# scheckmedia/centernet-uda

Hardware: AMD Instinct MI355X
Metric: images/sec CenterNet DLA-34 512x512 UDA step (entropy minimisation) (higher is better)
Workload: dtype f32; 1 GPU; configs[2]: DLA-34 + DCNv2, 512x512, per-GPU batch 16 source + 16 target, uda=entropy_minimization, Adam(lr 5e-5), random-init weights; global_batch=16, parallelism=dp1

## Files before the change

### centernet-uda_amd/csrc/dcn.hip

```cpp
#include <algorithm>
#include "igemm.cuh"
#include "igemm_host.h"

namespace cnuda {
namespace {

struct DcnGeom {
    int B, C, H, W, Co, kh, kw, sh, sw, ph, pw, dh, dw, dg, Ho, Wo;
    int off_bs, mask_bs, goff_bs, gmask_bs, gmask_logit;
};

struct Tap {
    int o00, o01, o10, o11;
    int h0, w0;
    float lh, lw, hh, hw;
    float mask;
    bool inside, c00, c01, c10, c11;
};

struct TapRaw { float dy, dx, mask; };
__device__ __forceinline__ TapRaw load_tap_raw(const DcnGeom& g, const float* __restrict__ off_b,
                                               const float* __restrict__ mask_b, int grp, int tap, int p) {
    const int T = g.kh * g.kw, HoWo = g.Ho * g.Wo;
    TapRaw r;
// ... 167 lines not shown
            if (k < K) {
                const int tap = k / g.C, c = k - tap * g.C;
                if (tap != cur) set_tap(tap);
                v = sample(in_b + (size_t)c * HW);
            }
            r.t[j].l = v;
        }
    }
    __device__ __forceinline__ void finish(const Raw& r, float (&v)[8]) {
        if (!r.eager) {
            if (!r.live) {
#pragma unroll
                for (int j = 0; j < 8; ++j) v[j] = 0.0f;
                return;
            }
#pragma unroll
            for (int j = 0; j < 8; ++j) v[j] = m00 * r.t[j].l + m01 * r.t[j].r + m10 * r.b[j].l + m11 * r.b[j].r;
            if constexpr (BUF) {
                if (col_on && col_voff != IG_BUF_OOB) {
                    const int k0s = __builtin_amdgcn_readfirstlane(r.k0);
                    const char* cbase = reinterpret_cast<const char*>(col_base);
                    unsigned voff = col_voff;
                    asm volatile("" : "+v"(voff));
#pragma unroll
                    for (int j = 0; j < 8; ++j) {
                        const size_t row = (size_t)(unsigned)((k0s + 2 * j) * col_stride) * 4u;
                        unsigned long long rbase = reinterpret_cast<unsigned long long>(cbase) + row;
                        asm volatile("" : "+s"(rbase));
                        *reinterpret_cast<__attribute__((address_space(1))) float*>(rbase + (unsigned long long)voff) = v[j];
                    }
                }
                return;
            }
            if (col_n) {
                float* cp = col_n + (size_t)r.k0 * col_stride;
                const size_t step = (size_t)2 * col_stride;
#pragma unroll
                for (int j = 0; j < 8; ++j) cp[j * step] = v[j];
            }
            return;
        }
#pragma unroll
        for (int j = 0; j < 8; ++j) {
            const int k = r.k0 + 2 * j;
            v[j] = r.t[j].l;
            if (col_n && k < K) col_n[(size_t)k * col_stride] = v[j];
        }
    }
    struct Out {
        float* base;
        int HoWo;
        __device__ Out(const Params& p, long long n) {
            HoWo = p.g.Ho * p.g.Wo;
            const int ni = (int)n, b = ni / HoWo, pp = ni - b * HoWo;
            base = p.out + (size_t)b * p.g.Co * HoWo + pp;
        }
        __device__ __forceinline__ void store(const Params& p, int m, float v) {
            v += p.bias[m];
            if (p.act_slope >= 0.0f && v < 0.0f) v *= p.act_slope;
            base[(size_t)m * HoWo] = v;
        }
        static constexpr bool kVec4 = true;
        __device__ static bool vec4_ok(const Params& p) { return ((p.g.Ho * p.g.Wo) & 3) == 0; }
        __device__ __forceinline__ void store4(const Params& p, int m, f32x4 v) {
            v += p.bias[m];
            if (p.act_slope >= 0.0f) {
#pragma unroll
                for (int e = 0; e < 4; ++e) if (v[e] < 0.0f) v[e] *= p.act_slope;
            }
            *reinterpret_cast<f32x4*>(base + (size_t)m * HoWo) = v;
        }
    };
};

using DcnFwdLoader = DcnFwdLoaderT<false>;
using DcnFwdBufLoader = DcnFwdLoaderT<true>;

constexpr int DW_MARGIN = 3;
typedef __attribute__((address_space(3))) volatile unsigned char lds_vu8;
template <int TC> struct DwTile {
    static constexpr int TR = IG_BN / TC, NR = TR + 2 + 2 * DW_MARGIN, RS = TC + 8, PL = NR * RS;
    static constexpr int CPR = TC / 4 + 2, CPP = NR * CPR, CELLS = 16 * CPP;
    static constexpr int NCELL = (CELLS + IG_THREADS - 1) / IG_THREADS;
    static constexpr int SHIFT = TC == 32 ? 5 : 4;
};
template <int TC> constexpr size_t dcnw_lds_floats(int bm) { return (size_t)16 * DwTile<TC>::PL + 2 * IG_KC * bm; }

template <int BM, int TC>
__global__ __launch_bounds__(IG_THREADS, 3) void dcnw_fwd_kernel(DcnFwdParams p, const float* __restrict__ A, int Mp, int Kp,
                                                                 int n_tiles, int tiles_x) {
    using Q = DwTile<TC>;
    constexpr int TM = BM / 32, PL = Q::PL, RS = Q::RS;
    extern __shared__ __attribute__((aligned(16))) float smem[];
    const DcnGeom& g = p.g;
    const int W = g.W, H = g.H, HW = g.H * g.W;
    float* const Hs = smem;
    float* const Asb = smem + 16 * PL;
    const int tid = threadIdx.x, lane = tid & 63, wid = tid >> 6;
    int tile = xcd_remap(blockIdx.x, n_tiles);
    const int tile_id = tile;
    const int tx = tile % tiles_x; tile /= tiles_x;
    const int tiles_y = H / Q::TR;
    const int ty = tile % tiles_y, b = tile / tiles_y;
    const int y0 = ty * Q::TR, x0 = tx * TC;
    const int yw0 = y0 - 1 - DW_MARGIN;
    const int pxl = wid * 32 + (lane & 31), kl = lane >> 5;
    const int py = y0 + (pxl >> Q::SHIFT), px = x0 + (pxl & (TC - 1)), pp = py * W + px;

    const buf_rsrc rs = ig_make_rsrc(p.in, (unsigned)((size_t)g.B * g.C * HW * sizeof(float)));
    auto cell = [&](int i, unsigned& voff, int& loff) {
        int salt = 0;
        asm volatile("" : "+v"(salt));
        const int e = tid + i * IG_THREADS + salt;
        const int c = e / Q::CPP, rem = e - c * Q::CPP;
        const int row = rem / Q::CPR, q4 = rem - row * Q::CPR;
        const int iy = yw0 + row, ix = x0 - 4 + 4 * q4;
        loff = e < Q::CELLS ? c * PL + row * RS + 4 * q4 : -1;
        voff = (e < Q::CELLS && iy >= 0 && iy < H && ix >= 0 && ix < W)
                   ? (unsigned)(((b * g.C + c) * HW + iy * W + ix) * (int)sizeof(float)) : IG_BUF_OOB;
    };

    int addr[9];
    float flh[9], flw[9], fmk[9];
    unsigned stray = 0;
    {
        const float* off_b = p.off + (size_t)b * g.off_bs + pp;
        const float* mask_b = p.mask + (size_t)b * g.mask_bs + pp;
        float dy[9], dx[9], mk[9];
#pragma unroll
        for (int t = 0; t < 9; ++t) {
            dy[t] = off_b[(size_t)(2 * t) * HW];
            dx[t] = off_b[(size_t)(2 * t + 1) * HW];
            mk[t] = mask_b[(size_t)t * HW];
        }
#pragma unroll
        for (int t = 0; t < 9; ++t) {
            const float h = (float)(py - 1 + t / 3) + dy[t], w = (float)(px - 1 + t % 3) + dx[t];
            const float hf = floorf(h), wf = floorf(w);
            const bool valid = h > -1.0f && w > -1.0f && h < (float)H && w < (float)W;
            const int h0 = valid ? (int)hf : 0, w0i = valid ? (int)wf : 0;
            const int wr = h0 - yw0, wc = w0i - x0 + 4;
            const bool inwin = valid && wr >= 0 && wr + 1 <= Q::NR - 1 && wc >= 0 && wc + 1 <= RS - 1;
            addr[t] = inwin ? wr * RS + wc : 0;
            flh[t] = h - hf;
            flw[t] = w - wf;
            fmk[t] = inwin ? mk[t] : 0.0f;
            if (valid && !inwin) stray |= 1u << t;
        }
    }
    const bool any_stray = __any(stray != 0);

    f32x16 acc[TM];
#pragma unroll
    for (int i = 0; i < TM; ++i)
#pragma unroll
        for (int r = 0; r < 16; ++r) acc[i][r] = 0.0f;

    f32x4 hreg[Q::NCELL];
    auto win_load = [&](int grp) {
        const unsigned soff = (unsigned)(grp * 16 * HW) * (unsigned)sizeof(float);
#pragma unroll
        for (int i = 0; i < Q::NCELL; ++i) {
            unsigned voff; int loff;
            cell(i, voff, loff);
            hreg[i] = ig_buf_load4(rs, voff, soff);
        }
    };
    auto win_store = [&]() {
#pragma unroll
        for (int i = 0; i < Q::NCELL; ++i) {
            unsigned voff; int loff;
            cell(i, voff, loff);
            if (loff >= 0) *reinterpret_cast<f32x4*>(Hs + loff) = hreg[i];
        }
    };
    f32x4 ra[ig_a_per<BM>()];
    const IgABuf<BM> abuf(A, Mp, Kp, 0, tid);
    const int nchunk = Kp / IG_KC, G = g.C >> 4;
    const bool col_on = p.col != nullptr;
    float* const col_l = col_on ? p.col + (size_t)b * 9 * g.C * HW + (size_t)kl * HW + pp : nullptr;

    win_load(0);
    abuf.load(0, ra);
    win_store();
    ig_store_a<BM>(Asb, tid, ra);
    if (1 < nchunk) abuf.load(IG_KC, ra);
    __syncthreads();
    int grp = 0;
    for (int c0 = 0; c0 < nchunk; c0 += 9, ++grp) {
        const bool more = grp + 1 < G;
        if (more) win_load(grp + 1);
#pragma unroll
        for (int t = 0; t < 9; ++t) {
            const int c = c0 + t;
            f32x4 ra2[ig_a_per<BM>()];
            if (c + 2 < nchunk) abuf.load((c + 2) * IG_KC, ra2);
            const float* As = Asb + (c & 1) * IG_KC * BM;
            const float* ap = As + kl * BM + (lane & 31);
            int a_t = addr[t];
            asm volatile("" : "+v"(a_t));
            const float* hb = Hs + kl * PL + a_t;
            const float lh = flh[t], lw = flw[t], hh = 1.0f - lh, hw = 1.0f - lw, mk = fmk[t];
            const float w00 = hh * hw * mk, w01 = hh * lw * mk, w10 = lh * hw * mk, w11 = lh * lw * mk;
            float v[IG_KC / 2], cr[IG_KC / 4][4];
            float* cp = nullptr;
            if (col_on) {
                unsigned long long rowoff = (unsigned long long)(unsigned)((t * g.C + grp * 16) * HW) * sizeof(float);
                asm volatile("" : "+s"(rowoff));
                cp = reinterpret_cast<float*>(reinterpret_cast<char*>(col_l) + rowoff);
            }
            auto read_half = [&](int h) {
#pragma unroll
                for (int s = 0; s < IG_KC / 4; ++s) {
                    const float* q = hb + 2 * (h * (IG_KC / 4) + s) * PL;
                    cr[s][0] = q[0]; cr[s][1] = q[1]; cr[s][2] = q[RS]; cr[s][3] = q[RS + 1];
                }
            };
            auto blend_half = [&](int h) {
#pragma unroll
                for (int s = 0; s < IG_KC / 4; ++s) {
                    float x = w00 * cr[s][0];
                    x = fmaf(w01, cr[s][1], x);
                    x = fmaf(w10, cr[s][2], x);
                    v[h * (IG_KC / 4) + s] = fmaf(w11, cr[s][3], x);
                }
                if (col_on) {
#pragma unroll
                    for (int s = 0; s < IG_KC / 4; ++s) cp[(size_t)(2 * (h * (IG_KC / 4) + s)) * HW] = v[h * (IG_KC / 4) + s];
                }
            };
            auto mma_half = [&](int h) {
#pragma unroll
                for (int s = h * (IG_KC / 4); s < (h + 1) * (IG_KC / 4); ++s) {
#pragma unroll
                    for (int i = 0; i < TM; ++i)
                        acc[i] = __builtin_amdgcn_mfma_f32_32x32x2f32(ap[2 * s * BM + i * 32], v[s], acc[i], 0, 0, 0);
                }
            };
            read_half(0);
            blend_half(0);
            read_half(1);
            __builtin_amdgcn_sched_barrier(0);
            mma_half(0);
            __builtin_amdgcn_sched_barrier(0);
            blend_half(1);
            mma_half(1);
            if (c + 1 < nchunk) ig_store_a<BM>(Asb + ((c + 1) & 1) * IG_KC * BM, tid, ra);
#pragma unroll
            for (int i = 0; i < ig_a_per<BM>(); ++i) ra[i] = ra2[i];
            __syncthreads();
            __builtin_amdgcn_sched_barrier(0);
        }
        if (any_stray) {
#pragma unroll 1
            for (int t0 = 0; t0 < 9; ++t0) {
                int t = t0;
                asm volatile("" : "+s"(t));
                if (!__any((stray >> t) & 1u)) continue;
                float sv[IG_KC / 2];
#pragma unroll
                for (int s = 0; s < IG_KC / 2; ++s) sv[s] = 0.0f;
                if ((stray >> t) & 1u) {
                    const float* off_b = p.off + (size_t)b * g.off_bs + pp;
                    const int tr = t / 3;
                    const float sh_ = (float)(py - 1 + tr) + off_b[(size_t)(2 * t) * HW];
                    const float sw_ = (float)(px - 1 + t - 3 * tr) + off_b[(size_t)(2 * t + 1) * HW];
                    const float smk = p.mask[(size_t)b * g.mask_bs + (size_t)t * HW + pp];
                    const float shf = floorf(sh_), swf = floorf(sw_);
                    const int sh0 = (int)shf, sw0 = (int)swf;
                    const float slh = sh_ - shf, slw = sw_ - swf, shh = 1.0f - slh, shw = 1.0f - slw;
                    const bool top = sh0 >= 0, bot = sh0 + 1 <= H - 1, lef = sw0 >= 0, rig = sw0 + 1 <= W - 1;
                    const float g00 = (top && lef) ? shh * shw * smk : 0.0f, g01 = (top && rig) ? shh * slw * smk : 0.0f;
                    const float g10 = (bot && lef) ? slh * shw * smk : 0.0f, g11 = (bot && rig) ? slh * slw * smk : 0.0f;
                    const int cy0 = top ? sh0 : 0, cy1 = bot ? sh0 + 1 : H - 1, cx0 = lef ? sw0 : 0, cx1 = rig ? sw0 + 1 : W - 1;
                    const float* in_c = p.in + ((size_t)b * g.C + grp * 16 + kl) * HW;
                    const int o00 = cy0 * W + cx0, o01 = cy0 * W + cx1, o10 = cy1 * W + cx0, o11 = cy1 * W + cx1;
#pragma unroll
                    for (int s = 0; s < IG_KC / 2; ++s) {
                        const float* pl = in_c + (size_t)(2 * s) * HW;
                        float x = g00 * pl[o00];
                        x = fmaf(g01, pl[o01], x);
                        x = fmaf(g10, pl[o10], x);
                        sv[s] = fmaf(g11, pl[o11], x);
                    }
                    if (col_on) {
                        float* cp = col_l + (size_t)(t * g.C + grp * 16) * HW;
#pragma unroll
                        for (int s = 0; s < IG_KC / 2; ++s) cp[(size_t)(2 * s) * HW] = sv[s];
                    }
                }
                const float* ag = A + (size_t)((c0 + t) * IG_KC + kl) * Mp + (lane & 31);
#pragma unroll
                for (int s = 0; s < IG_KC / 2; ++s) {
#pragma unroll
                    for (int i = 0; i < TM; ++i)
                        acc[i] = __builtin_amdgcn_mfma_f32_32x32x2f32(ag[(size_t)(2 * s) * Mp + i * 32], sv[s], acc[i], 0, 0, 0);
                }
            }
        }
        if (more) {
            win_store();
            __syncthreads();
        }
    }
    float* stage = smem + wid * IG_EPI_WAVE;
    const int col = lane & 31, cg = lane & 7, rsub = lane >> 3;
    const int epl = wid * 32 + 4 * cg;
    float* const obase = p.out + (size_t)b * g.Co * HW + (size_t)(y0 + (epl >> Q::SHIFT)) * W + x0 + (epl & (TC - 1));
#pragma unroll
    for (int i = 0; i < TM; ++i) {
#pragma unroll
        for (int r = 0; r < 16; ++r) stage[mfma_row(r, lane) * IG_EPI_LD + col] = acc[i][r];
        asm volatile("s_waitcnt lgkmcnt(0)" ::: "memory");
#pragma unroll
        for (int it = 0; it < 4; ++it) {
            const int row = it * 8 + rsub;
            f32x4 v4 = *reinterpret_cast<const f32x4*>(stage + row * IG_EPI_LD + 4 * cg);
            const int m = i * 32 + row;
            if (m < g.Co) {
                v4 += p.bias[m];
                if (p.act_slope >= 0.0f) {
#pragma unroll
                    for (int e = 0; e < 4; ++e) if (v4[e] < 0.0f) v4[e] *= p.act_slope;
                }
                *reinterpret_cast<f32x4*>(obase + (size_t)m * HW) = v4;
            }
            if (p.stats) {
                float s1 = (v4[0] + v4[1]) + (v4[2] + v4[3]);
                float s2 = (v4[0] * v4[0] + v4[1] * v4[1]) + (v4[2] * v4[2] + v4[3] * v4[3]);
                auto row8 = [](float v) {
                    v += __builtin_bit_cast(float, __builtin_amdgcn_update_dpp(0, __builtin_bit_cast(int, v), 0xB1, 0xf, 0xf, false));
                    v += __builtin_bit_cast(float, __builtin_amdgcn_update_dpp(0, __builtin_bit_cast(int, v), 0x4E, 0xf, 0xf, false));
                    v += __builtin_bit_cast(float, __builtin_amdgcn_update_dpp(0, __builtin_bit_cast(int, v), 0x141, 0xf, 0xf, false));
                    return v;
                };
                s1 = row8(s1);
                s2 = row8(s2);
                if (cg == 0)
                    reinterpret_cast<float2*>(p.stats)[((size_t)tile_id * 4 + wid) * p.stats_mp + m] = make_float2(s1, s2);
            }
        }
        asm volatile("s_waitcnt lgkmcnt(0)" ::: "memory");
    }
}

struct DcnSampleParams {
    DcnGeom g;
    const float *in, *off, *mask;
    float* col;
};
__global__ __launch_bounds__(1024) void dcn_sample_kernel(DcnSampleParams p, int tiles_per_image) {
    const DcnGeom& g = p.g;
    const int T = g.kh * g.kw, HoWo = g.Ho * g.Wo, HW = g.H * g.W;
    const int b = blockIdx.x / tiles_per_image, tile = blockIdx.x - b * tiles_per_image;
    const int px = tile * 64 + threadIdx.x;
    if (px >= HoWo) return;
    const int oy = px / g.Wo, ox = px - oy * g.Wo;
    const float* in_b = p.in + (size_t)b * g.C * HW;
    for (int tap = threadIdx.y; tap < T; tap += blockDim.y) {
        const Tap t = make_tap(g, p.off + (size_t)b * g.off_bs, p.mask + (size_t)b * g.mask_bs, 0, tap, oy, ox);
        const float mk = t.inside ? t.mask : 0.0f;
        const float w00 = t.c00 ? t.hh * t.hw * mk : 0.0f, w01 = t.c01 ? t.hh * t.lw * mk : 0.0f;
        const float w10 = t.c10 ? t.lh * t.hw * mk : 0.0f, w11 = t.c11 ? t.lh * t.lw * mk : 0.0f;
        float* dst = p.col + ((size_t)b * T + tap) * g.C * HoWo + px;
        const bool paired = g.W >= 2;
        const bool ledge = t.w0 < 0, redge = t.w0 > g.W - 2;
        const int wa = ledge ? 0 : (redge ? g.W - 2 : t.w0);
        const int ht = t.h0 < 0 ? 0 : t.h0, hb = t.h0 + 1 > g.H - 1 ? g.H - 1 : t.h0 + 1;
        const int qT = t.inside ? ht * g.W + wa : 0, qB = t.inside ? hb * g.W + wa : 0;
        for (int c0 = 0; c0 < g.C; c0 += 8) {
            float e00[8], e01[8], e10[8], e11[8];
            if (paired) {
                Pair pt[8], pb[8];
#pragma unroll
                for (int u = 0; u < 8; ++u) {
                    const float* plane = in_b + (size_t)(c0 + u < g.C ? c0 + u : g.C - 1) * HW;
                    pt[u] = *reinterpret_cast<const Pair*>(plane + qT);
                    pb[u] = *reinterpret_cast<const Pair*>(plane + qB);
                }
#pragma unroll
                for (int u = 0; u < 8; ++u) {
                    e00[u] = redge ? pt[u].r : pt[u].l; e01[u] = ledge ? pt[u].l : pt[u].r;
                    e10[u] = redge ? pb[u].r : pb[u].l; e11[u] = ledge ? pb[u].l : pb[u].r;
                }
            } else {
#pragma unroll
                for (int u = 0; u < 8; ++u) {
                    const float* plane = in_b + (size_t)(c0 + u < g.C ? c0 + u : g.C - 1) * HW;
                    e00[u] = plane[t.o00]; e01[u] = plane[t.o01]; e10[u] = plane[t.o10]; e11[u] = plane[t.o11];
                }
// ... 924 lines not shown
}

extern "C" int cnuda_dcn_v2_forward(const float* input, const float* weight, const float* bias, const float* offset,
                                    const float* mask, float* output, int B, int C, int H, int W, int Cout, int kh,
                                    int kw, int sh, int sw, int ph, int pw, int dh, int dw, int dg, void* workspace,
                                    size_t workspace_bytes, cnuda_stream_t stream) {
    return cnuda_dcn_v2_forward_cols(input, weight, bias, offset, mask, output, nullptr, B, C, H, W, Cout, kh, kw, sh,
                                     sw, ph, pw, dh, dw, dg, workspace, workspace_bytes, stream);
}

extern "C" int cnuda_dcn_v2_forward_cols(const float* input, const float* weight, const float* bias,
                                         const float* offset, const float* mask, float* output, float* columns, int B,
                                         int C, int H, int W, int Cout, int kh, int kw, int sh, int sw, int ph, int pw,
                                         int dh, int dw, int dg, void* workspace, size_t workspace_bytes,
                                         cnuda_stream_t stream) {
    return cnuda_dcn_v2_forward_act(input, weight, bias, offset, mask, output, columns, -1.0f, B, C, H, W, Cout, kh, kw,
                                    sh, sw, ph, pw, dh, dw, dg, workspace, workspace_bytes, stream);
}

extern "C" int cnuda_dcn_v2_stats_block(int B, int C, int H, int W, int Cout, int kh, int kw, int sh, int sw, int ph, int pw,
                                        int dh, int dw, int dg, int* rows) {
    DcnGeom g;
    if (fill_geom(g, B, C, H, W, Cout, kh, kw, sh, sw, ph, pw, dh, dw, dg, "cnuda_dcn_v2_stats_block")) return 0;
    return plan_stats_block(g, make_plan(g), rows);
}

static int dcn_forward_impl(const DcnFwdCall& c, const DcnPlan& q) {
    const DcnGeom& g = c.g;
    CNUDA_REQUIRE(c.input && c.weight && c.bias && c.offset && c.mask && c.output, "cnuda_dcn_v2_forward: null pointer");
    CNUDA_REQUIRE(!c.columns || g.W >= 2, "cnuda_dcn_v2_forward_cols: columns output needs width >= 2");
    hipStream_t st = (hipStream_t)c.stream;
    CNUDA_REQUIRE(c.act_slope < 0.0f || (g.dg == 1 && g.W >= 2), "cnuda_dcn_v2_forward_act: fused activation needs deformable_group == 1 and width >= 2");
    if (q.fwd == DcnFwdPath::Composed) {
        const int Cg = g.C / g.dg, T = q.T, HoWo = g.Ho * g.Wo;
        const long long HW = (long long)g.H * g.W;
        const size_t inner = cnuda_dcn_v2_workspace_bytes(g.B, Cg, g.H, g.W, g.Co, g.kh, g.kw, g.sh, g.sw, g.ph, g.pw, g.dh, g.dw, 1);
        Carver cv(c.workspace, c.workspace_bytes);
        float* xg = cv.take<float>((size_t)g.B * Cg * HW);
        float* wg = cv.take<float>((size_t)g.Co * Cg * T);
        float* tmp = cv.take<float>((size_t)g.B * g.Co * HoWo);
        float* zero = cv.take<float>((size_t)g.Co);
        void* iws = cv.take<char>(inner);
        CNUDA_REQUIRE(c.workspace && cv.cur <= cv.end, "cnuda_dcn_v2_forward: workspace too small");
        if (hipMemsetAsync(zero, 0, (size_t)g.Co * sizeof(float), st) != hipSuccess) return check_launch("cnuda_dcn_v2_forward(dg>1)");
        DcnFwdCall gc = c;
        gc.g.C = Cg; gc.g.dg = 1;
        gc.input = xg; gc.weight = wg;
        gc.workspace = iws; gc.workspace_bytes = inner;
        const DcnPlan gq = make_plan(gc.g);
        const PackStampSuspend uncached;
        for (int grp = 0; grp < g.dg; ++grp) {
            if (int rc = cnuda_copy_channels(c.input, xg, g.B, Cg, HW, g.C, grp * Cg, Cg, 0, c.stream)) return rc;
            if (int rc = cnuda_copy_channels(c.weight, wg, g.Co, Cg, T, g.C, grp * Cg, Cg, 0, c.stream)) return rc;
            gc.bias = grp == 0 ? c.bias : zero;
            gc.offset = c.offset + (size_t)grp * 2 * T * HoWo;
            gc.mask = c.mask + (size_t)grp * T * HoWo;
            gc.output = grp == 0 ? c.output : tmp;
            gc.columns = c.columns ? c.columns + (size_t)grp * g.B * T * Cg * HoWo : nullptr;
            if (int rc = dcn_forward_impl(gc, gq)) return rc;
            if (grp > 0)
                if (int rc = cnuda_add(c.output, tmp, c.output, (long long)g.B * g.Co * HoWo, c.stream)) return rc;
        }
        return check_launch("cnuda_dcn_v2_forward(dg>1)");
    }
    if (q.fwd == DcnFwdPath::Naive) {
        DcnNaiveParams p{g, c.input, c.weight, c.bias, c.offset, c.mask, nullptr, c.output, nullptr, nullptr, nullptr, nullptr};
        CNUDA_LAUNCH(dcn_naive_fwd_kernel, dim3(stream_grid((long long)g.B * g.Co * g.Ho * g.Wo, 256)), dim3(256),
                           0, st, p);
        return check_launch("cnuda_dcn_v2_forward(dg>1)");
    }
    CNUDA_REQUIRE(q.N < (1ll << 31) - IG_BN, "cnuda_dcn_v2_forward: more than 2^31 pixels per call");
    CNUDA_REQUIRE(c.workspace && c.workspace_bytes >= q.fwd_bytes, "cnuda_dcn_v2_forward: workspace too small");
    Carver cv(c.workspace, c.workspace_bytes);
    if (q.fwd == DcnFwdPath::Window) {
        const int bm = 64;
        const float* Aw = launch_pack(c.weight, cv.take<float>((size_t)q.Kp * bm), (size_t)q.Kp * bm * sizeof(float), g.Co, g.C,
                                      q.T, PACK_HALO_FWD, q.Kp, bm, 0, st);
        DcnFwdParams p{g, c.input, c.offset, c.mask, c.bias, c.act_slope, c.output, c.columns, c.stats, 64};
        ProfScope prof(st);
        prof.name("dcnw_fwd_kernel<%d>%s", bm, c.columns ? " (+ column side output)" : "");
        const int tiles_x = g.W / dcnw_tile_cols(g.W), n_tiles = (int)(q.N / IG_BN);
        bool lds_ok = true;
        const bool found = with_tiles<Tile<64, 32>, Tile<64, 16>>(bm, dcnw_tile_cols(g.W), [&](auto BM, auto TC) {
            const size_t fl = dcnw_lds_floats<TC()>(BM());
            const size_t lds = (fl < (size_t)4 * IG_EPI_WAVE ? (size_t)4 * IG_EPI_WAVE : fl) * sizeof(float);
            lds_ok = raise_dynamic_lds(reinterpret_cast<const void*>(&dcnw_fwd_kernel<BM(), TC()>), lds);
            if (lds_ok) CNUDA_LAUNCH((dcnw_fwd_kernel<BM(), TC()>), dim3(n_tiles), dim3(IG_THREADS), lds, st, p, Aw, bm, q.Kp, n_tiles, tiles_x);
        });
        CNUDA_REQUIRE(lds_ok, "cnuda_dcn_v2_forward: dynamic LDS");
        CNUDA_REQUIRE(found, "cnuda_dcn_v2_forward: no dcnw_fwd_kernel instance for %d-column tiles", dcnw_tile_cols(g.W));
        return check_launch("cnuda_dcn_v2_forward(window)");
    }
    const float* A = launch_pack(c.weight, cv.take<float>((size_t)q.Kp * q.Mp), (size_t)q.Kp * q.Mp * sizeof(float), g.Co,
                                 g.C, q.T, PACK_FWD, q.Kp, q.Mp, 0, st);
    if (q.fwd == DcnFwdPath::SampleThenGemm) {
        float* cols = c.columns ? c.columns : cv.take<float>((size_t)g.B * q.K * g.Ho * g.Wo);
        ProfScope prof(st);
        prof.name("dcn_sample_kernel + igemm_fwd_kernel<%d, DcnColsLoader>", q.bm);
        {
            DcnSampleParams sp{g, c.input, c.offset, c.mask, cols};
            const int tiles = ceil_div(g.Ho * g.Wo, 64), tw = q.T < 16 ? q.T : 16;
            CNUDA_LAUNCH(dcn_sample_kernel, dim3(g.B * tiles), dim3(64, tw), 0, st, sp, tiles);
        }
        DcnColsParams p{g, cols, c.bias, c.act_slope, c.output, c.stats, q.Mp};
        const bool found = q.fwd_ws    ? launch_dcn_fwd<DcnColsBufLoader, true>(q, p, A, g.Co, st)
                           : q.fwd_buf ? launch_dcn_fwd<DcnColsBufLoader>(q, p, A, g.Co, st)
                                       : launch_dcn_fwd<DcnColsLoader>(q, p, A, g.Co, st);
        CNUDA_REQUIRE(found, "cnuda_dcn_v2_forward: no GEMM instance for a %d-row tile", q.bm);
        return check_launch("cnuda_dcn_v2_forward(columns + GEMM)");
    }
    DcnFwdParams p{g, c.input, c.offset, c.mask, c.bias, c.act_slope, c.output, c.columns, c.stats, q.Mp};
    ProfScope prof(st);
    prof.name("igemm_fwd_kernel<%d, DcnFwdLoader>%s", q.bm, c.columns ? " (+ column side output)" : "");
    const bool found = q.fwd_buf ? launch_dcn_fwd<DcnFwdBufLoader>(q, p, A, g.Co, st) : launch_dcn_fwd<DcnFwdLoader>(q, p, A, g.Co, st);
    CNUDA_REQUIRE(found, "cnuda_dcn_v2_forward: no GEMM instance for a %d-row tile", q.bm);
    return check_launch("cnuda_dcn_v2_forward");
}

extern "C" int cnuda_dcn_v2_forward_act(const float* input, const float* weight, const float* bias,
                                        const float* offset, const float* mask, float* output, float* columns,
                                        float act_slope, int B, int C, int H, int W, int Cout, int kh, int kw, int sh,
                                        int sw, int ph, int pw, int dh, int dw, int dg, void* workspace,
                                        size_t workspace_bytes, cnuda_stream_t stream) {
    DcnFwdCall c{};
    if (int rc = fill_geom(c.g, B, C, H, W, Cout, kh, kw, sh, sw, ph, pw, dh, dw, dg, "cnuda_dcn_v2_forward")) return rc;
    c.input = input; c.weight = weight; c.bias = bias; c.offset = offset; c.mask = mask;
    c.output = output; c.columns = columns; c.act_slope = act_slope;
    c.workspace = workspace; c.workspace_bytes = workspace_bytes; c.stream = stream;
    return dcn_forward_impl(c, make_plan(c.g));
}

extern "C" int cnuda_dcn_v2_forward_stats(const float* input, const float* weight, const float* bias,
                                          const float* offset, const float* mask, float* output, float* columns,
                                          float* stats, int stats_block, int stats_rows, int B, int C, int H, int W,
                                          int Cout, int kh, int kw, int sh,
                                          int sw, int ph, int pw, int dh, int dw, int dg, void* workspace,
                                          size_t workspace_bytes, cnuda_stream_t stream) {
    DcnFwdCall c{};
    if (int rc = fill_geom(c.g, B, C, H, W, Cout, kh, kw, sh, sw, ph, pw, dh, dw, dg, "cnuda_dcn_v2_forward")) return rc;
    const DcnPlan q = make_plan(c.g);
    if (stats) {
        int rows = 0;
        const int blk = plan_stats_block(c.g, q, &rows);
        CNUDA_REQUIRE(blk != 0, "cnuda_dcn_v2_forward_stats: no statistics for this call (cnuda_dcn_v2_stats_block says which)");
        CNUDA_REQUIRE(blk == stats_block && rows == stats_rows,
                      "cnuda_dcn_v2_forward_stats: the statistics buffer was sized for blocks of %d pixels x %d rows, this call "
                      "writes %d x %d (did the offset regime change between cnuda_dcn_v2_stats_block and the call?)",
                      stats_block, stats_rows, blk, rows);
    }
    c.input = input; c.weight = weight; c.bias = bias; c.offset = offset; c.mask = mask;
    c.output = output; c.columns = columns; c.stats = stats; c.act_slope = -1.0f;
    c.workspace = workspace; c.workspace_bytes = workspace_bytes; c.stream = stream;
    return dcn_forward_impl(c, q);
}

extern "C" int cnuda_dcn_v2_forward_om(const float* input, const float* weight, const float* bias, const float* om,
                                       float* output, float* columns, float* stats, int stats_block, int stats_rows,
                                       float act_slope, int B,
                                       int C, int H, int W, int Cout, int kh, int kw, int sh, int sw, int ph, int pw, int dh,
                                       int dw, int dg, void* workspace, size_t workspace_bytes, cnuda_stream_t stream) {
    CNUDA_REQUIRE(om && dg == 1 && W >= 2, "cnuda_dcn_v2_forward_om: needs deformable_group == 1 and width >= 2");
    DcnFwdCall c{};
    if (int rc = fill_geom(c.g, B, C, H, W, Cout, kh, kw, sh, sw, ph, pw, dh, dw, dg, "cnuda_dcn_v2_forward_om")) return rc;
    const DcnPlan q = make_plan(c.g);
    if (stats) {
        int rows = 0;
        const int blk = plan_stats_block(c.g, q, &rows);
        CNUDA_REQUIRE(blk != 0 && blk == stats_block && rows == stats_rows,
// ... 212 lines not shown
```

### centernet-uda_amd/csrc/igemm.cuh

```cuda
#pragma once
#include <type_traits>
#include <utility>
#include "common.h"
#include "igemm_host.h"

namespace cnuda {

using f32x16 = __attribute__((ext_vector_type(16))) float;

constexpr int IG_BN = 128;
constexpr int IG_BK = 16;
constexpr int IG_KC = 16;
constexpr int IG_THREADS = 256;

template <int BM> struct IgTile;
template <> struct IgTile<128> { static constexpr int WM = 2, WN = 2, TM = 2, TN = 2; };
template <> struct IgTile<64>  { static constexpr int WM = 2, WN = 2, TM = 1, TN = 2; };
template <> struct IgTile<32>  { static constexpr int WM = 1, WN = 4, TM = 1, TN = 1; };

__device__ __forceinline__ int xcd_remap(int bid, int nwg) {
    constexpr int NX = 8;
    const int per = nwg / NX, rem = nwg % NX;
    const int x = bid % NX, q = bid / NX;
    const int start = x * per + (x < rem ? x : rem);
// ... 105 lines not shown
template <int BM>
__device__ __forceinline__ void ig_mma_frag_x3(const u32x4 (&a)[IgTile<BM>::TM][3], const u32x4 (&b)[IgTile<BM>::TN][3],
                                               f32x16 (&acc)[IgTile<BM>::TM][IgTile<BM>::TN]) {
    using T = IgTile<BM>;
    auto mm = [&](const u32x4& x, const u32x4& y, f32x16& c) {
        c = __builtin_amdgcn_mfma_f32_32x32x16_bf16(__builtin_bit_cast(bf16x8, x), __builtin_bit_cast(bf16x8, y), c, 0, 0, 0);
    };
#pragma unroll
    for (int t = 0; t < 6; ++t) {
        constexpr int qa[6] = {2, 1, 0, 1, 0, 0}, qb[6] = {0, 1, 2, 0, 1, 0};
#pragma unroll
        for (int i = 0; i < T::TM; ++i)
#pragma unroll
            for (int j = 0; j < T::TN; ++j) mm(a[i][qa[t]], b[j][qb[t]], acc[i][j]);
    }
}

template <int BM> constexpr int ig_a3_per() { return (6 * BM + IG_THREADS - 1) / IG_THREADS; }
template <int BM>
__device__ __forceinline__ void ig_load_a_x3(const u32x4* __restrict__ A3, int Mp, int k0, int m0, int tid,
                                             u32x4 (&r)[ig_a3_per<BM>()]) {
    const u32x4* base = A3 + (size_t)(k0 >> 4) * 6 * Mp + m0;
#pragma unroll
    for (int i = 0; i < ig_a3_per<BM>(); ++i) {
        const int e = tid + i * IG_THREADS;
        const int ec = (6 * BM) % IG_THREADS == 0 ? e : (e < 6 * BM ? e : e % (6 * BM));
        r[i] = base[(size_t)(ec / BM) * Mp + ec % BM];
    }
}
template <int BM>
__device__ __forceinline__ void ig_store_a_x3(u32x4* __restrict__ As, int tid, const u32x4 (&r)[ig_a3_per<BM>()]) {
#pragma unroll
    for (int i = 0; i < ig_a3_per<BM>(); ++i) {
        const int e = tid + i * IG_THREADS;
        if ((6 * BM) % IG_THREADS == 0 || e < 6 * BM) As[e] = r[i];
    }
}
static __global__ void split_a_kernel(const float* __restrict__ A, u32x4* __restrict__ A3, int Kp, int Mp) {
    const long long total = (long long)(Kp / 16) * 2 * Mp;
    for (long long i = (long long)blockIdx.x * blockDim.x + threadIdx.x; i < total; i += (long long)gridDim.x * blockDim.x) {
        const int m = (int)(i % Mp), h = (int)(i / Mp) & 1, c = (int)(i / (2 * Mp));
        float v[8];
#pragma unroll
        for (int j = 0; j < 8; ++j) v[j] = A[(size_t)(16 * c + h + 2 * j) * Mp + m];
        unsigned o[3][4];
        x3_split<8>(v, o);
#pragma unroll
        for (int q = 0; q < 3; ++q) A3[((size_t)(c * 3 + q) * 2 + h) * Mp + m] = u32x4{o[q][0], o[q][1], o[q][2], o[q][3]};
    }
}
inline size_t ig_a_bytes(size_t Kp, size_t Mp) { return Kp * Mp * 10; }

using f32x4 = __attribute__((ext_vector_type(4))) float;
template <int BM, int KC = IG_KC> constexpr int ig_a_per() { return (BM * KC / 4 + IG_THREADS - 1) / IG_THREADS; }
template <int BM, int KC = IG_KC>
__device__ __forceinline__ void ig_load_a(const float* __restrict__ A, int Mp, int k0, int m0, int tid,
                                          f32x4 (&r)[ig_a_per<BM, KC>()]) {
    constexpr int CELLS = BM * KC / 4;
#pragma unroll
    for (int i = 0; i < ig_a_per<BM, KC>(); ++i) {
        const int e = tid + i * IG_THREADS;
        const int ec = CELLS % IG_THREADS == 0 ? e : (e < CELLS ? e : e - CELLS);
        const int kk = ec / (BM / 4), m = (ec % (BM / 4)) * 4;
        r[i] = *reinterpret_cast<const f32x4*>(A + (size_t)(k0 + kk) * Mp + m0 + m);
    }
}
template <int BM, int KC = IG_KC>
__device__ __forceinline__ void ig_store_a(float* __restrict__ As, int tid, const f32x4 (&r)[ig_a_per<BM, KC>()]) {
    constexpr int CELLS = BM * KC / 4;
#pragma unroll
    for (int i = 0; i < ig_a_per<BM, KC>(); ++i) {
        const int e = tid + i * IG_THREADS;
        if (CELLS % IG_THREADS == 0 || e < CELLS) reinterpret_cast<f32x4*>(As)[e] = r[i];
    }
}

using buf_rsrc = __amdgpu_buffer_rsrc_t;
constexpr unsigned IG_BUF_OOB = 0x80000000u;
__device__ __forceinline__ buf_rsrc ig_make_rsrc(const void* base, unsigned bytes) {
    return __builtin_amdgcn_make_buffer_rsrc(const_cast<void*>(base), 0, (int)bytes, 0x00020000);
}
__device__ __forceinline__ float ig_buf_load(buf_rsrc r, unsigned voff, unsigned soff) {
    return __builtin_bit_cast(float, __builtin_amdgcn_raw_buffer_load_b32(r, (int)voff, (int)soff, 0));
}
__device__ __forceinline__ f32x4 ig_buf_load4(buf_rsrc r, unsigned voff, unsigned soff) {
    return __builtin_bit_cast(f32x4, __builtin_amdgcn_raw_buffer_load_b128(r, (int)voff, (int)soff, 0));
}
template <int BM, int KC = IG_KC>
struct IgABuf {
    buf_rsrc rs;
    unsigned voff[ig_a_per<BM, KC>()];
    int Mp;
    __device__ __forceinline__ IgABuf(const float* A, int Mp_, int Kp, int m0, int tid) : Mp(Mp_) {
        rs = ig_make_rsrc(A + m0, (unsigned)(((size_t)Kp * Mp_ - m0) * sizeof(float)));
        constexpr int CELLS = BM * KC / 4;
#pragma unroll
        for (int i = 0; i < ig_a_per<BM, KC>(); ++i) {
            const int e = tid + i * IG_THREADS;
            const int ec = CELLS % IG_THREADS == 0 ? e : (e < CELLS ? e : e - CELLS);
            voff[i] = (unsigned)(((ec / (BM / 4)) * Mp_ + (ec % (BM / 4)) * 4) * (int)sizeof(float));
        }
    }
    __device__ __forceinline__ void load(int k0, f32x4 (&r)[ig_a_per<BM, KC>()]) const {
        const unsigned soff = (unsigned)(k0 * Mp) * (unsigned)sizeof(float);
#pragma unroll
        for (int i = 0; i < ig_a_per<BM, KC>(); ++i) r[i] = ig_buf_load4(rs, voff[i], soff);
    }
};


constexpr int IG_EPI_LD = 36;
constexpr int IG_EPI_WAVE = 32 * IG_EPI_LD;
template <class P, class = void> struct IgHasStats : std::false_type {};
template <class P> struct IgHasStats<P, std::void_t<decltype(std::declval<P>().stats)>> : std::true_type {};
template <int BM> constexpr int ig_stat_px() { return IgTile<BM>::TN * 32; }
template <int BM, class Loader>
__device__ __forceinline__ void ig_epilogue_vec4(const typename Loader::Params& p, float* __restrict__ stage,
                                                 const f32x16 (&acc)[IgTile<BM>::TM][IgTile<BM>::TN], int m0, long long n0,
                                                 int wm_off, int wn_off, int lane, int M, long long N) {
    using T = IgTile<BM>;
    const int col = lane & 31, cg = lane & 7, rsub = lane >> 3;
    constexpr bool kStats = IgHasStats<typename Loader::Params>::value;
    bool stats_on = false;
    if constexpr (kStats) stats_on = p.stats != nullptr;
    float ssum[T::TM][4], ssq[T::TM][4];
#pragma unroll
    for (int i = 0; i < T::TM; ++i)
#pragma unroll
        for (int it = 0; it < 4; ++it) { ssum[i][it] = 0.0f; ssq[i][it] = 0.0f; }
#pragma unroll
    for (int j = 0; j < T::TN; ++j) {
        const long long n = n0 + wn_off + j * 32 + 4 * cg;
        typename Loader::Out out(p, n < N ? n : 0);
#pragma unroll
        for (int i = 0; i < T::TM; ++i) {
#pragma unroll
            for (int r = 0; r < 16; ++r) stage[mfma_row(r, lane) * IG_EPI_LD + col] = acc[i][j][r];
            asm volatile("s_waitcnt lgkmcnt(0)" ::: "memory");
#pragma unroll
            for (int it = 0; it < 4; ++it) {
                const int row = it * 8 + rsub;
                const f32x4 v = *reinterpret_cast<const f32x4*>(stage + row * IG_EPI_LD + 4 * cg);
                const int m = m0 + wm_off + i * 32 + row;
                if (m < M && n < N) out.store4(p, m, v);
                if constexpr (kStats) {
                    if (stats_on) {
                        f32x4 w = v;
                        if (p.bias && m < M) w += p.bias[m];
                        if (!(n < N)) w = f32x4{0.f, 0.f, 0.f, 0.f};
                        ssum[i][it] += (w[0] + w[1]) + (w[2] + w[3]);
                        ssq[i][it] += (w[0] * w[0] + w[1] * w[1]) + (w[2] * w[2] + w[3] * w[3]);
                    }
                }
            }
            asm volatile("s_waitcnt lgkmcnt(0)" ::: "memory");
        }
    }
    if constexpr (kStats) {
        if (stats_on) {
            auto row8 = [](float v) {
                v += __builtin_bit_cast(float, __builtin_amdgcn_update_dpp(0, __builtin_bit_cast(int, v), 0xB1, 0xf, 0xf, false));
                v += __builtin_bit_cast(float, __builtin_amdgcn_update_dpp(0, __builtin_bit_cast(int, v), 0x4E, 0xf, 0xf, false));
                v += __builtin_bit_cast(float, __builtin_amdgcn_update_dpp(0, __builtin_bit_cast(int, v), 0x141, 0xf, 0xf, false));
                return v;
            };
            const long long blk = (n0 + wn_off) / ig_stat_px<BM>();
// ... 675 lines not shown
```

Before: 220.6 images/sec.

## Stream DCN window weights from global into registers and split next-window prefetch

The windowed deformable-conv forward kernel stops staging the weight (A) chunks through double-buffered LDS with a barrier per chunk. Each lane now loads its MFMA A fragments directly from global memory into registers via buffer loads, one chunk ahead. The next channel-group window is fetched in two halves, with the first half parked in LDS, to cut register pressure. Column writes become buffer stores. This removes nine block-wide barriers per group and frees LDS, in exchange for more scalar global loads per lane and an extra LDS park/unpark pass.

```diff
diff --git a/centernet-uda_amd/csrc/dcn.hip b/centernet-uda_amd/csrc/dcn.hip
--- a/centernet-uda_amd/csrc/dcn.hip
+++ b/centernet-uda_amd/csrc/dcn.hip
@@ -273,9 +273,14 @@
     static constexpr int TR = IG_BN / TC, NR = TR + 2 + 2 * DW_MARGIN, RS = TC + 8, PL = NR * RS;
     static constexpr int CPR = TC / 4 + 2, CPP = NR * CPR, CELLS = 16 * CPP;
     static constexpr int NCELL = (CELLS + IG_THREADS - 1) / IG_THREADS;
+    static constexpr int NH = NCELL / 2;
+    static_assert(NCELL % 2 == 0, "the next window arrives in two halves");
     static constexpr int SHIFT = TC == 32 ? 5 : 4;
 };
-template <int TC> constexpr size_t dcnw_lds_floats(int bm) { return (size_t)16 * DwTile<TC>::PL + 2 * IG_KC * bm; }
+template <int TC> constexpr size_t dcnw_lds_floats() {
+    constexpr size_t fl = (size_t)16 * DwTile<TC>::PL + (size_t)DwTile<TC>::NH * IG_THREADS * 4;
+    return fl > (size_t)4 * IG_EPI_WAVE ? fl : (size_t)4 * IG_EPI_WAVE;
+}
 
 template <int BM, int TC>
 __global__ __launch_bounds__(IG_THREADS, 3) void dcnw_fwd_kernel(DcnFwdParams p, const float* __restrict__ A, int Mp, int Kp,
@@ -286,7 +291,7 @@
     const DcnGeom& g = p.g;
     const int W = g.W, H = g.H, HW = g.H * g.W;
     float* const Hs = smem;
-    float* const Asb = smem + 16 * PL;
+    f32x4* const Ps = reinterpret_cast<f32x4*>(smem + 16 * PL);
     const int tid = threadIdx.x, lane = tid & 63, wid = tid >> 6;
     int tile = xcd_remap(blockIdx.x, n_tiles);
     const int tile_id = tile;
@@ -347,66 +352,103 @@
 #pragma unroll
         for (int r = 0; r < 16; ++r) acc[i][r] = 0.0f;
 
-    f32x4 hreg[Q::NCELL];
-    auto win_load = [&](int grp) {
+    constexpr int NH = Q::NH;
+    f32x4 hreg[NH];
+    auto win_load = [&](int grp, int half, f32x4 (&r)[NH]) {
         const unsigned soff = (unsigned)(grp * 16 * HW) * (unsigned)sizeof(float);
 #pragma unroll
-        for (int i = 0; i < Q::NCELL; ++i) {
+        for (int i = 0; i < NH; ++i) {
+            unsigned voff; int loff;
+            cell(half * NH + i, voff, loff);
+            r[i] = ig_buf_load4(rs, voff, soff);
+        }
+    };
+    auto win_store = [&](int half, const f32x4 (&r)[NH]) {
+#pragma unroll
+        for (int i = 0; i < NH; ++i) {
+            unsigned voff; int loff;
+            cell(half * NH + i, voff, loff);
+            if (loff >= 0) *reinterpret_cast<f32x4*>(Hs + loff) = r[i];
+        }
+    };
+    auto win_park = [&]() {
+#pragma unroll
+        for (int i = 0; i < NH; ++i) Ps[i * IG_THREADS + tid] = hreg[i];
+    };
+    auto win_unpark = [&]() {
+#pragma unroll
+        for (int i = 0; i < NH; ++i) {
             unsigned voff; int loff;
             cell(i, voff, loff);
-            hreg[i] = ig_buf_load4(rs, voff, soff);
+            const f32x4 r = Ps[i * IG_THREADS + tid];
+            if (loff >= 0) *reinterpret_cast<f32x4*>(Hs + loff) = r;
         }
     };
-    auto win_store = [&]() {
-#pragma unroll
-        for (int i = 0; i < Q::NCELL; ++i) {
-            unsigned voff; int loff;
-            cell(i, voff, loff);
-            if (loff >= 0) *reinterpret_cast<f32x4*>(Hs + loff) = hreg[i];
-        }
+    static_assert((IG_KC * BM) * sizeof(float) <= 4096, "a chunk's fragment offsets fit the buffer instruction's immediate");
+    constexpr int AH = (IG_KC / 4) * TM;
+    const buf_rsrc ars = ig_make_rsrc(A, (unsigned)((size_t)Kp * BM * sizeof(float)));
+    float af[2][AH];
+    auto a_load = [&](int c, int h) {
+        unsigned soff = (unsigned)(c * IG_KC * BM) * (unsigned)sizeof(float);
+        asm volatile("" : "+s"(soff));
+        unsigned l = (unsigned)tid;
+        asm volatile("" : "+v"(l));
+        const unsigned vo = (((l >> 5) & 1u) * BM + (l & 31u)) * (unsigned)sizeof(float);
+#pragma unroll
+        for (int s = 0; s < IG_KC / 4; ++s)
+#pragma unroll
+            for (int i = 0; i < TM; ++i)
+                af[h][s * TM + i] = ig_buf_load(ars, vo + (unsigned)((2 * (h * (IG_KC / 4) + s) * BM + i * 32) * (int)sizeof(float)), soff);
     };
-    f32x4 ra[ig_a_per<BM>()];
-    const IgABuf<BM> abuf(A, Mp, Kp, 0, tid);
     const int nchunk = Kp / IG_KC, G = g.C >> 4;
     const bool col_on = p.col != nullptr;
-    float* const col_l = col_on ? p.col + (size_t)b * 9 * g.C * HW + (size_t)kl * HW + pp : nullptr;
-
-    win_load(0);
-    abuf.load(0, ra);
-    win_store();
-    ig_store_a<BM>(Asb, tid, ra);
-    if (1 < nchunk) abuf.load(IG_KC, ra);
+    const float* const col_b = p.col + (size_t)b * 9 * g.C * HW;
+    const unsigned col_bytes = col_on ? (unsigned)(g.C * HW) * (unsigned)sizeof(float) : 0u;
+    const unsigned col_voff = (unsigned)(kl * HW + pp) * (unsigned)sizeof(float);
+
+    {
+        f32x4 h1[NH];
+        win_load(0, 0, hreg);
+        win_load(0, 1, h1);
+        a_load(0, 0);
+        a_load(0, 1);
+        win_store(0, hreg);
+        win_store(1, h1);
+    }
     __syncthreads();
     int grp = 0;
     for (int c0 = 0; c0 < nchunk; c0 += 9, ++grp) {
         const bool more = grp + 1 < G;
-        if (more) win_load(grp + 1);
-#pragma unroll
-        for (int t = 0; t < 9; ++t) {
-            const int c = c0 + t;
-            f32x4 ra2[ig_a_per<BM>()];
-            if (c + 2 < nchunk) abuf.load((c + 2) * IG_KC, ra2);
-            const float* As = Asb + (c & 1) * IG_KC * BM;
-            const float* ap = As + kl * BM + (lane & 31);
+        float cr[IG_KC / 4][4];
+        auto read_half = [&](int t, int h) {
             int a_t = addr[t];
             asm volatile("" : "+v"(a_t));
             const float* hb = Hs + kl * PL + a_t;
-            const float lh = flh[t], lw = flw[t], hh = 1.0f - lh, hw = 1.0f - lw, mk = fmk[t];
+#pragma unroll
+            for (int s = 0; s < IG_KC / 4; ++s) {
+                const float* q = hb + 2 * (h * (IG_KC / 4) + s) * PL;
+                cr[s][0] = q[0]; cr[s][1] = q[1]; cr[s][2] = q[RS]; cr[s][3] = q[RS + 1];
+            }
+        };
+        read_half(0, 0);
+#pragma unroll
+        for (int t = 0; t < 9; ++t) {
+            const int c = c0 + t;
+            if (more && t == 0) win_load(grp + 1, 0, hreg);
+            if (more && t == 2) {
+                win_park();
+                win_load(grp + 1, 1, hreg);
+            }
+            float lh = flh[t], lw = flw[t], mk = fmk[t];
+            asm volatile("" : "+v"(lh), "+v"(lw), "+v"(mk));
+            const float hh = 1.0f - lh, hw = 1.0f - lw;
             const float w00 = hh * hw * mk, w01 = hh * lw * mk, w10 = lh * hw * mk, w11 = lh * lw * mk;
-            float v[IG_KC / 2], cr[IG_KC / 4][4];
-            float* cp = nullptr;
-            if (col_on) {
-                unsigned long long rowoff = (unsigned long long)(unsigned)((t * g.C + grp * 16) * HW) * sizeof(float);
-                asm volatile("" : "+s"(rowoff));
-                cp = reinterpret_cast<float*>(reinterpret_cast<char*>(col_l) + rowoff);
-            }
-            auto read_half = [&](int h) {
-#pragma unroll
-                for (int s = 0; s < IG_KC / 4; ++s) {
-                    const float* q = hb + 2 * (h * (IG_KC / 4) + s) * PL;
-                    cr[s][0] = q[0]; cr[s][1] = q[1]; cr[s][2] = q[RS]; cr[s][3] = q[RS + 1];
-                }
-            };
+            float v[IG_KC / 2];
+            unsigned long long tapoff = (unsigned long long)t * (unsigned)(g.C * HW) * sizeof(float);
+            asm volatile("" : "+s"(tapoff));
+            const buf_rsrc crs = ig_make_rsrc(reinterpret_cast<const char*>(col_b) + tapoff, col_bytes);
+            unsigned crow = (unsigned)(grp * 16 * HW) * (unsigned)sizeof(float);
+            asm volatile("" : "+s"(crow));
             auto blend_half = [&](int h) {
 #pragma unroll
                 for (int s = 0; s < IG_KC / 4; ++s) {
@@ -415,31 +457,35 @@
                     x = fmaf(w10, cr[s][2], x);
                     v[h * (IG_KC / 4) + s] = fmaf(w11, cr[s][3], x);
                 }
-                if (col_on) {
-#pragma unroll
-                    for (int s = 0; s < IG_KC / 4; ++s) cp[(size_t)(2 * (h * (IG_KC / 4) + s)) * HW] = v[h * (IG_KC / 4) + s];
+            };
+            auto store_half = [&](int h) {
+#pragma unroll
+                for (int s = 0; s < IG_KC / 4; ++s)
+                    ig_buf_store(crs, col_voff, crow + (unsigned)(2 * (h * (IG_KC / 4) + s) * HW) * (unsigned)sizeof(float), v[h * (IG_KC / 4) + s]);
+            };
+            auto mma_half = [&](int h) {
+#pragma unroll
+                for (int s = h * (IG_KC / 4); s < (h + 1) * (IG_KC / 4); ++s) {
+#pragma unroll
+                    for (int i = 0; i < TM; ++i)
+                        acc[i] = __builtin_amdgcn_mfma_f32_32x32x2f32(af[h][(s - h * (IG_KC / 4)) * TM + i], v[s], acc[i], 0, 0, 0);
                 }
             };
-            auto mma_half = [&](int h) {
-#pragma unroll
-                for (int s = h * (IG_KC / 4); s < (h + 1) * (IG_KC / 4); ++s) {
-#pragma unroll
-                    for (int i = 0; i < TM; ++i)
-                        acc[i] = __builtin_amdgcn_mfma_f32_32x32x2f32(ap[2 * s * BM + i * 32], v[s], acc[i], 0, 0, 0);
-                }
-            };
-            read_half(0);
             blend_half(0);
-            read_half(1);
+            read_half(t, 1);
             __builtin_amdgcn_sched_barrier(0);
             mma_half(0);
             __builtin_amdgcn_sched_barrier(0);
+            const int cn = c + 1 < nchunk ? c + 1 : c;
+            a_load(cn, 0);
+            store_half(0);
             blend_half(1);
+            if (t + 1 < 9) read_half(t + 1, 0);
+            __builtin_amdgcn_sched_barrier(0);
             mma_half(1);
-            if (c + 1 < nchunk) ig_store_a<BM>(Asb + ((c + 1) & 1) * IG_KC * BM, tid, ra);
-#pragma unroll
-            for (int i = 0; i < ig_a_per<BM>(); ++i) ra[i] = ra2[i];
-            __syncthreads();
+            __builtin_amdgcn_sched_barrier(0);
+            a_load(cn, 1);
+            store_half(1);
             __builtin_amdgcn_sched_barrier(0);
         }
         if (any_stray) {
@@ -475,6 +521,7 @@
                         sv[s] = fmaf(g11, pl[o11], x);
                     }
                     if (col_on) {
+                        float* const col_l = p.col + (size_t)b * 9 * g.C * HW + (size_t)kl * HW + pp;
                         float* cp = col_l + (size_t)(t * g.C + grp * 16) * HW;
 #pragma unroll
                         for (int s = 0; s < IG_KC / 2; ++s) cp[(size_t)(2 * s) * HW] = sv[s];
@@ -489,14 +536,18 @@
                 }
             }
         }
+        __syncthreads();
         if (more) {
-            win_store();
+            win_store(1, hreg);
+            win_unpark();
             __syncthreads();
         }
     }
     float* stage = smem + wid * IG_EPI_WAVE;
     const int col = lane & 31, cg = lane & 7, rsub = lane >> 3;
-    const int epl = wid * 32 + 4 * cg;
+    int te = tid;
+    asm volatile("" : "+v"(te));
+    const int epl = (te >> 6) * 32 + 4 * (te & 7);
     float* const obase = p.out + (size_t)b * g.Co * HW + (size_t)(y0 + (epl >> Q::SHIFT)) * W + x0 + (epl & (TC - 1));
 #pragma unroll
     for (int i = 0; i < TM; ++i) {
@@ -1587,8 +1638,7 @@
         const int tiles_x = g.W / dcnw_tile_cols(g.W), n_tiles = (int)(q.N / IG_BN);
         bool lds_ok = true;
         const bool found = with_tiles<Tile<64, 32>, Tile<64, 16>>(bm, dcnw_tile_cols(g.W), [&](auto BM, auto TC) {
-            const size_t fl = dcnw_lds_floats<TC()>(BM());
-            const size_t lds = (fl < (size_t)4 * IG_EPI_WAVE ? (size_t)4 * IG_EPI_WAVE : fl) * sizeof(float);
+            const size_t lds = dcnw_lds_floats<TC()>() * sizeof(float);
             lds_ok = raise_dynamic_lds(reinterpret_cast<const void*>(&dcnw_fwd_kernel<BM(), TC()>), lds);
             if (lds_ok) CNUDA_LAUNCH((dcnw_fwd_kernel<BM(), TC()>), dim3(n_tiles), dim3(IG_THREADS), lds, st, p, Aw, bm, q.Kp, n_tiles, tiles_x);
         });
diff --git a/centernet-uda_amd/csrc/igemm.cuh b/centernet-uda_amd/csrc/igemm.cuh
--- a/centernet-uda_amd/csrc/igemm.cuh
+++ b/centernet-uda_amd/csrc/igemm.cuh
@@ -211,6 +211,9 @@
 }
 __device__ __forceinline__ float ig_buf_load(buf_rsrc r, unsigned voff, unsigned soff) {
     return __builtin_bit_cast(float, __builtin_amdgcn_raw_buffer_load_b32(r, (int)voff, (int)soff, 0));
+}
+__device__ __forceinline__ void ig_buf_store(buf_rsrc r, unsigned voff, unsigned soff, float v) {
+    __builtin_amdgcn_raw_buffer_store_b32(__builtin_bit_cast(unsigned, v), r, (int)voff, (int)soff, 0);
 }
 __device__ __forceinline__ f32x4 ig_buf_load4(buf_rsrc r, unsigned voff, unsigned soff) {
     return __builtin_bit_cast(f32x4, __builtin_amdgcn_raw_buffer_load_b128(r, (int)voff, (int)soff, 0));
```

After: 221.9 images/sec (median of 6 runs). No clear change (+0.6%).
